# SparkJiao/llama-pipeline-parallel

Measured on AMD Instinct MI355X. Metric: tokens/sec (whole node), LLaMA-65B PP=8 seq4096 at 1/2/4/8 MI355X, higher is better.
Workload: dtype bf16; 1 GPU; model=llama-65b, measured_model=llama-65b-shaped 10-layer slice (10/80 layers), global_batch=64, seq_len=4096, parallelism=pp1, num_layers=10, micro_batch_size=4, grad_accum_steps=16

## Files before the change

### lpp_amd/ops/csrc/attention_bwd.hip

```cpp
#include "common.h"
#include "attn_order.h"

namespace lpp {

typedef __attribute__((ext_vector_type(8))) short bf16x8;
typedef __attribute__((ext_vector_type(16))) float f32x16;
typedef __attribute__((ext_vector_type(2))) int int2v;

constexpr int AB_D = 128;

__device__ __forceinline__ int bswz(int row, int col_elem) {
  return row * 256 + ((col_elem * 2) ^ ((row & 15) << 4));
}
__device__ __forceinline__ unsigned cvt_pk_bf16_(float lo, float hi) {
  unsigned r;
  asm("v_cvt_pk_bf16_f32 %0, %1, %2" : "=v"(r) : "v"(lo), "v"(hi));
  return r;
}
__device__ __forceinline__ float bf2f_(short s) {
  union { unsigned u; float f; } cv;
  cv.u = ((unsigned)(unsigned short)s) << 16;
  return cv.f;
}
__device__ __forceinline__ short f2bf_(float f) {
  __hip_bfloat16 h = __float2bfloat16(f);
  return *reinterpret_cast<short*>(&h);
}

__device__ __forceinline__ void quad_transpose(const bf16x8& v, int st_r, int out[4]) {
#pragma unroll
  for (int k = 0; k < 4; ++k) out[k] = reinterpret_cast<const int*>(&v)[k];
  {
    int t0 = __shfl_xor(out[(st_r & 1) ^ 1], 16);
    int t1 = __shfl_xor(out[((st_r & 1) ^ 1) | 2], 16);
    if (st_r & 1) { out[0] = t0; out[2] = t1; } else { out[1] = t0; out[3] = t1; }
  }
  {
    int lo = (st_r & 2) ? 0 : 2;
    int t0 = __shfl_xor(out[lo], 32);
    int t1 = __shfl_xor(out[lo + 1], 32);
    out[lo] = t0; out[lo + 1] = t1;
  }
}

__device__ __forceinline__ int tswz(int d, int r) {
  return (d * 64 + (r ^ ((((d >> 3) ^ d) & 7) << 3))) * 2;
}

__device__ __forceinline__ void write_transposed(char* img, int r0, int d0,
                                                 const int dw[4]) {
#pragma unroll
  for (int e = 0; e < 2; ++e) {
    const int d = d0 + e;
    unsigned w01 = e ? (((unsigned)dw[0] >> 16) | ((unsigned)dw[1] & 0xffff0000u))
                     : (((unsigned)dw[0] & 0xffffu) | ((unsigned)dw[1] << 16));
    unsigned w23 = e ? (((unsigned)dw[2] >> 16) | ((unsigned)dw[3] & 0xffff0000u))
                     : (((unsigned)dw[2] & 0xffffu) | ((unsigned)dw[3] << 16));
    int2v pair = {(int)w01, (int)w23};
    *reinterpret_cast<int2v*>(img + tswz(d, r0)) = pair;
  }
}

__device__ __forceinline__ void pack_pair(const float p[16], bf16x8 out[2]) {
#pragma unroll
  for (int ksl = 0; ksl < 2; ++ksl) {
    const float* pr = &p[8 * ksl];
    const unsigned x1 = cvt_pk_bf16_(pr[0], pr[1]);
    const unsigned x2 = cvt_pk_bf16_(pr[2], pr[3]);
    const unsigned y1 = cvt_pk_bf16_(pr[4], pr[5]);
    const unsigned y2 = cvt_pk_bf16_(pr[6], pr[7]);
    const int2v a = __builtin_amdgcn_permlane32_swap((int)x1, (int)y1, false, false);
    const int2v b = __builtin_amdgcn_permlane32_swap((int)x2, (int)y2, false, false);
    int w[4] = {a[0], b[0], a[1], b[1]};
    out[ksl] = *reinterpret_cast<const bf16x8*>(w);
  }
}

__global__ __launch_bounds__(256) void attn_bwd_delta_kernel(
    const short* __restrict__ dO, const short* __restrict__ O,
    float* __restrict__ delta, int64_t rows, int S, int H) {
  const int lg = threadIdx.x & 15;
  const int grp = (blockIdx.x * 256 + (int)threadIdx.x) >> 4;
  const int64_t stride = ((int64_t)gridDim.x * 256) >> 4;
  for (int64_t r = grp; r < rows; r += stride) {
    const bf16x8 d8 = *reinterpret_cast<const bf16x8*>(&dO[r * AB_D + lg * 8]);
    const bf16x8 o8 = *reinterpret_cast<const bf16x8*>(&O[r * AB_D + lg * 8]);
    float acc = 0.f;
#pragma unroll
    for (int j = 0; j < 8; ++j) acc += bf2f_(d8[j]) * bf2f_(o8[j]);
#pragma unroll
    for (int m = 1; m < 16; m <<= 1) acc += __shfl_xor(acc, m);
    if (lg == 0) {
      const int h = (int)(r % H);
      const int64_t bs = r / H;
      const int s = (int)(bs % S);
      const int64_t b = bs / S;
      delta[(b * H + h) * S + s] = acc;
    }
  }
}

constexpr int DQ_QW = 32, DQ_WAVES = 8, DQ_QB = 256, DQ_KVB = 64;

template <bool DBUF>
__global__ __launch_bounds__(512, 2) void attn_bwd_dq_kernel(
    const short* __restrict__ Q, const short* __restrict__ K,
    const short* __restrict__ V, const short* __restrict__ dO,
    const float* __restrict__ LSE2, const float* __restrict__ Delta,
    short* __restrict__ dQ,
    int B, int S, int H, int HKV, float c, float scale,
    int order_mode, int order_G) {
  extern __shared__ __attribute__((aligned(16))) char smem[];
  constexpr int NB = DBUF ? 2 : 1;
  auto k_lds = [&](int buf) -> char* { return smem + (DBUF ? buf : 0) * 16384; };
  auto v_lds = [&](int buf) -> char* {
    return smem + NB * 16384 + (DBUF ? buf : 0) * 16384; };
  auto kt_lds = [&](int buf) -> char* {
    return smem + 2 * NB * 16384 + (DBUF ? buf : 0) * 16384; };

  const int tid = threadIdx.x;
  const int wid = tid >> 6;
  const int lane = tid & 63;
  const int lq = lane & 31;
  const int hi2 = lane >> 5;

  const AttnBlock ob = attn_block_order(blockIdx.x, (S + DQ_QB - 1) / DQ_QB, B * H,
                                        order_G, ATTN_ORDER_FWD_DQ, order_mode);
  const int qblk = ob.blk;
  const int b = ob.head / H;
  const int h = ob.head % H;
  const int hkv = h / (H / HKV);
  const int64_t sHD = (int64_t)H * AB_D;
  const int64_t sHkvD = (int64_t)HKV * AB_D;
  const int64_t q_base = (((int64_t)b * S) * H + h) * AB_D;
  const int64_t kv_base = (((int64_t)b * S) * HKV + hkv) * AB_D;
  const int64_t ld_base = ((int64_t)b * H + h) * S;

  const int qw0 = qblk * DQ_QB + wid * DQ_QW;
  const int qrow = qw0 + lq;

  bf16x8 qf[8], dof[8];
  {
    const int64_t rb = q_base + (int64_t)min(qrow, S - 1) * sHD;
#pragma unroll
    for (int dc = 0; dc < 8; ++dc) {
      qf[dc] = *reinterpret_cast<const bf16x8*>(&Q[rb + dc * 16 + hi2 * 8]);
      dof[dc] = *reinterpret_cast<const bf16x8*>(&dO[rb + dc * 16 + hi2 * 8]);
    }
  }
  const float Lq = LSE2[ld_base + min(qrow, S - 1)];
  const float Dq = Delta[ld_base + min(qrow, S - 1)];

  const int st_r = lane >> 4;
  const int st_c = 8 * (lane & 15);
  const int kv_end = min(S, (qblk + 1) * DQ_QB);

  auto ld_tile = [&](int kv0, int pass, bf16x8& kreg, bf16x8& vreg) {
    const int row = min(kv0 + 4 * wid + 32 * pass + st_r, S - 1);
    const int64_t rb = kv_base + (int64_t)row * sHkvD + st_c;
    kreg = *reinterpret_cast<const bf16x8*>(&K[rb]);
    vreg = *reinterpret_cast<const bf16x8*>(&V[rb]);
  };
  auto write_tile = [&](int buf, int pass, bf16x8 kreg, bf16x8 vreg) {
    const int r = 4 * wid + 32 * pass + st_r;
    *reinterpret_cast<bf16x8*>(k_lds(buf) + bswz(r, st_c)) = kreg;
    *reinterpret_cast<bf16x8*>(v_lds(buf) + bswz(r, st_c)) = vreg;
    int dw[4];
    quad_transpose(kreg, st_r, dw);
    write_transposed(kt_lds(buf), 4 * wid + 32 * pass, st_c + 2 * st_r, dw);
  };

  f32x16 dq_acc[4];
#pragma unroll
  for (int dt = 0; dt < 4; ++dt)
#pragma unroll
    for (int r = 0; r < 16; ++r) dq_acc[dt][r] = 0.f;

  bf16x8 kreg0, kreg1, vreg0, vreg1;
  ld_tile(0, 0, kreg0, vreg0);
  ld_tile(0, 1, kreg1, vreg1);
  write_tile(0, 0, kreg0, vreg0);
  write_tile(0, 1, kreg1, vreg1);
  if (DBUF && DQ_KVB < kv_end) {
    ld_tile(DQ_KVB, 0, kreg0, vreg0);
    ld_tile(DQ_KVB, 1, kreg1, vreg1);
  }
  __syncthreads();

  for (int kv0 = 0, cur = 0; kv0 < kv_end; kv0 += DQ_KVB, cur ^= 1) {
    const bool have_next = kv0 + DQ_KVB < kv_end;
    if (DBUF) {
      if (have_next) {
        write_tile(cur ^ 1, 0, kreg0, vreg0);
        write_tile(cur ^ 1, 1, kreg1, vreg1);
        if (kv0 + 2 * DQ_KVB < kv_end) {
          ld_tile(kv0 + 2 * DQ_KVB, 0, kreg0, vreg0);
          ld_tile(kv0 + 2 * DQ_KVB, 1, kreg1, vreg1);
        }
      }
    } else if (have_next) {
      ld_tile(kv0 + DQ_KVB, 0, kreg0, vreg0);
      ld_tile(kv0 + DQ_KVB, 1, kreg1, vreg1);
    }

    if (kv0 < qw0 + DQ_QW) {
      f32x16 st[2], dpt[2];
#pragma unroll
      for (int t2 = 0; t2 < 2; ++t2)
#pragma unroll
        for (int r = 0; r < 16; ++r) { st[t2][r] = 0.f; dpt[t2][r] = 0.f; }
      __builtin_amdgcn_s_setprio(1);
#pragma unroll
      for (int dc = 0; dc < 8; ++dc) {
#pragma unroll
        for (int t2 = 0; t2 < 2; ++t2) {
          const bf16x8 ak = *reinterpret_cast<const bf16x8*>(
              k_lds(cur) + bswz(t2 * 32 + lq, dc * 16 + hi2 * 8));
          const bf16x8 av = *reinterpret_cast<const bf16x8*>(
              v_lds(cur) + bswz(t2 * 32 + lq, dc * 16 + hi2 * 8));
          st[t2] = __builtin_amdgcn_mfma_f32_32x32x16_bf16(ak, qf[dc], st[t2], 0, 0, 0);
          dpt[t2] = __builtin_amdgcn_mfma_f32_32x32x16_bf16(av, dof[dc], dpt[t2], 0, 0, 0);
        }
      }
      __builtin_amdgcn_s_setprio(0);

      const bool need_mask = (kv0 + DQ_KVB > qw0) || (kv0 + DQ_KVB > S);
      float ds[32];
#pragma unroll
      for (int t2 = 0; t2 < 2; ++t2)
#pragma unroll
        for (int r = 0; r < 16; ++r) {
          bool ok = true;
          if (need_mask) {
            const int kv = kv0 + t2 * 32 + (r & 3) + 8 * (r >> 2) + 4 * hi2;
            ok = (kv <= qrow) && (kv < S);
          }
          const float p = ok ? exp2f(fmaf(st[t2][r], c, -Lq)) : 0.f;
          ds[t2 * 16 + r] = p * (dpt[t2][r] - Dq);
        }

      bf16x8 dsa[4];
      pack_pair(&ds[0], &dsa[0]);
      pack_pair(&ds[16], &dsa[2]);

      __builtin_amdgcn_s_setprio(1);
#pragma unroll
      for (int dt = 0; dt < 4; ++dt) {
        const int d = dt * 32 + lq;
#pragma unroll
        for (int ks = 0; ks < 4; ++ks) {
          const bf16x8 bk = *reinterpret_cast<const bf16x8*>(
              kt_lds(cur) + tswz(d, ks * 16 + hi2 * 8));
          dq_acc[dt] = __builtin_amdgcn_mfma_f32_32x32x16_bf16(dsa[ks], bk, dq_acc[dt], 0, 0, 0);
        }
      }
      __builtin_amdgcn_s_setprio(0);
    }

    if (!DBUF && have_next) {
      __syncthreads();
      write_tile(0, 0, kreg0, vreg0);
      write_tile(0, 1, kreg1, vreg1);
    }
    __syncthreads();
  }

#pragma unroll
  for (int r = 0; r < 16; ++r) {
    const int row = qw0 + (r & 3) + 8 * (r >> 2) + 4 * hi2;
    if (row >= S) continue;
    const int64_t rb = q_base + (int64_t)row * sHD;
#pragma unroll
    for (int dt = 0; dt < 4; ++dt) dQ[rb + dt * 32 + lq] = f2bf_(dq_acc[dt][r] * scale);
  }
}

constexpr int KV_KW = 16, KV_WG = 128, KV_QT = 64;
constexpr int TS40 = 40;

typedef __attribute__((ext_vector_type(4))) float f32x4;


__device__ __forceinline__ bf16x8 pack_frag16(const float p[2][4], int hi4_odd) {
  unsigned X0 = cvt_pk_bf16_(p[0][0], p[0][1]);
  unsigned Y0 = cvt_pk_bf16_(p[0][2], p[0][3]);
  unsigned X1 = cvt_pk_bf16_(p[1][0], p[1][1]);
  unsigned Y1 = cvt_pk_bf16_(p[1][2], p[1][3]);
  const int2v ax = __builtin_amdgcn_permlane32_swap((int)X0, (int)X1, false, false);
  const int2v cx = __builtin_amdgcn_permlane16_swap(ax[0], ax[0], false, false);
  const int2v cpx = __builtin_amdgcn_permlane16_swap(ax[1], ax[1], false, false);
  const int2v ay = __builtin_amdgcn_permlane32_swap((int)Y0, (int)Y1, false, false);
  const int2v cy = __builtin_amdgcn_permlane16_swap(ay[0], ay[0], false, false);
  const int2v cpy = __builtin_amdgcn_permlane16_swap(ay[1], ay[1], false, false);
  int w[4];
  w[0] = hi4_odd ? cpx[0] : ax[0];
  w[1] = hi4_odd ? cpy[0] : ay[0];
  w[2] = hi4_odd ? ax[1] : cx[1];
  w[3] = hi4_odd ? ay[1] : cy[1];
  return *reinterpret_cast<const bf16x8*>(w);
}

template <bool DBUF>
__global__ __launch_bounds__(512, 2) void attn_bwd_dkdv_kernel(
    const short* __restrict__ Q, const short* __restrict__ K,
    const short* __restrict__ V, const short* __restrict__ dO,
    const float* __restrict__ LSE2, const float* __restrict__ Delta,
    short* __restrict__ dK, short* __restrict__ dV,
    int B, int S, int H, int HKV, float c, float scale,
    int order_mode, int order_G) {
  extern __shared__ __attribute__((aligned(16))) char smem[];
  constexpr int NB = DBUF ? 2 : 1;
  auto q_lds = [&](int buf) -> char* { return smem + (DBUF ? buf : 0) * 16384; };
  auto do_lds = [&](int buf) -> char* {
    return smem + NB * 16384 + (DBUF ? buf : 0) * 16384; };
  auto qt_lds = [&](int buf) -> char* {
    return smem + 2 * NB * 16384 + (DBUF ? buf : 0) * 16384; };
  auto dot_lds = [&](int buf) -> char* {
    return smem + 3 * NB * 16384 + (DBUF ? buf : 0) * 16384; };
  auto l_buf = [&](int buf) -> float* {
    return reinterpret_cast<float*>(smem + 4 * NB * 16384) + (DBUF ? buf : 0) * 64; };
  auto d_buf = [&](int buf) -> float* {
    return reinterpret_cast<float*>(smem + 4 * NB * 16384 + NB * 256) +
           (DBUF ? buf : 0) * 64; };


  const int tid = threadIdx.x;
  const int wid = tid >> 6;
  const int lane = tid & 63;
  const int l16 = lane & 15;
  const int hi4 = (lane >> 4) & 3;

  const AttnBlock ob = attn_block_order(blockIdx.x, (S + KV_WG - 1) / KV_WG, B * HKV,
                                        order_G, ATTN_ORDER_DKDV, order_mode);
  const int kvblk = ob.blk;
  const int b = ob.head / HKV;
  const int hkv = ob.head % HKV;
  const int G = H / HKV;
  const int64_t sHD = (int64_t)H * AB_D;
  const int64_t sHkvD = (int64_t)HKV * AB_D;
  const int64_t kv_base = (((int64_t)b * S) * HKV + hkv) * AB_D;

  const int kvw0 = kvblk * KV_WG + wid * KV_KW;
  const int kvrow = kvw0 + l16;

  bf16x8 kf[4], vf[4];
  {
    const int64_t rb = kv_base + (int64_t)min(kvrow, S - 1) * sHkvD;
#pragma unroll
    for (int dc = 0; dc < 4; ++dc) {
      kf[dc] = *reinterpret_cast<const bf16x8*>(&K[rb + dc * 32 + hi4 * 8]);
      vf[dc] = *reinterpret_cast<const bf16x8*>(&V[rb + dc * 32 + hi4 * 8]);
    }
  }

  f32x4 dv_acc[8], dk_acc[8];
#pragma unroll
  for (int dt = 0; dt < 8; ++dt)
#pragma unroll
    for (int r = 0; r < 4; ++r) { dv_acc[dt][r] = 0.f; dk_acc[dt][r] = 0.f; }

  const int st_r = (lane >> 4) & 3;
  const int st_c = 8 * (lane & 15);
  const int qstart = kvblk * KV_WG;

  for (int g = 0; g < G; ++g) {
    const int h = hkv * G + g;
    const int64_t q_base = (((int64_t)b * S) * H + h) * AB_D;
    const int64_t ld_base = ((int64_t)b * H + h) * S;

    auto ld_tile = [&](int qt0, int pass, bf16x8& qreg, bf16x8& dreg) {
      const int row = min(qt0 + 4 * wid + 32 * pass + st_r, S - 1);
      const int64_t rb = q_base + (int64_t)row * sHD + st_c;
      qreg = *reinterpret_cast<const bf16x8*>(&Q[rb]);
      dreg = *reinterpret_cast<const bf16x8*>(&dO[rb]);
    };
    auto write_tile = [&](int buf, int qt0, int pass, bf16x8 qreg, bf16x8 dreg) {
      const int r = 4 * wid + 32 * pass + st_r;
      *reinterpret_cast<bf16x8*>(q_lds(buf) + bswz(r, st_c)) = qreg;
      *reinterpret_cast<bf16x8*>(do_lds(buf) + bswz(r, st_c)) = dreg;
      int dw[4];
      quad_transpose(qreg, st_r, dw);
      write_transposed(qt_lds(buf), r - st_r, st_c + 2 * st_r, dw);
      quad_transpose(dreg, st_r, dw);
      write_transposed(dot_lds(buf), r - st_r, st_c + 2 * st_r, dw);
      if (pass == 0 && tid < 128) {
        const int qi = min(qt0 + (tid & 63), S - 1);
        if (tid < 64) l_buf(buf)[tid] = LSE2[ld_base + qi];
        else d_buf(buf)[tid & 63] = Delta[ld_base + qi];
      }
    };

    bf16x8 qreg0, dreg0, qreg1, dreg1;
    ld_tile(qstart, 0, qreg0, dreg0);
    ld_tile(qstart, 1, qreg1, dreg1);
    write_tile(0, qstart, 0, qreg0, dreg0);
    write_tile(0, qstart, 1, qreg1, dreg1);
    if (DBUF && qstart + KV_QT < S) {
      ld_tile(qstart + KV_QT, 0, qreg0, dreg0);
      ld_tile(qstart + KV_QT, 1, qreg1, dreg1);
    }
    __syncthreads();

    for (int qt0 = qstart, cur = 0; qt0 < S; qt0 += KV_QT, cur ^= 1) {
      const bool have_next = qt0 + KV_QT < S;
      if (DBUF) {
        if (have_next) {
          write_tile(cur ^ 1, qt0 + KV_QT, 0, qreg0, dreg0);
          write_tile(cur ^ 1, qt0 + KV_QT, 1, qreg1, dreg1);
          if (qt0 + 2 * KV_QT < S) {
            ld_tile(qt0 + 2 * KV_QT, 0, qreg0, dreg0);
            ld_tile(qt0 + 2 * KV_QT, 1, qreg1, dreg1);
          }
        }
      } else if (have_next) {
        ld_tile(qt0 + KV_QT, 0, qreg0, dreg0);
        ld_tile(qt0 + KV_QT, 1, qreg1, dreg1);
      }

      if (qt0 + KV_QT - 1 >= kvw0) {
#pragma unroll
        for (int half = 0; half < 2; ++half) {
          const int qh0 = qt0 + half * 32;
          if (qh0 + 31 < kvw0) continue;
          f32x4 st[2], dpt[2];
#pragma unroll
          for (int qs = 0; qs < 2; ++qs)
#pragma unroll
            for (int r = 0; r < 4; ++r) { st[qs][r] = 0.f; dpt[qs][r] = 0.f; }
          __builtin_amdgcn_s_setprio(1);
#pragma unroll
          for (int dc = 0; dc < 4; ++dc) {
#pragma unroll
            for (int qs = 0; qs < 2; ++qs) {
              const bf16x8 aq = *reinterpret_cast<const bf16x8*>(
                  q_lds(cur) + bswz(half * 32 + qs * 16 + l16, dc * 32 + hi4 * 8));
              const bf16x8 ad = *reinterpret_cast<const bf16x8*>(
                  do_lds(cur) + bswz(half * 32 + qs * 16 + l16, dc * 32 + hi4 * 8));
              st[qs] = __builtin_amdgcn_mfma_f32_16x16x32_bf16(aq, kf[dc], st[qs], 0, 0, 0);
              dpt[qs] = __builtin_amdgcn_mfma_f32_16x16x32_bf16(ad, vf[dc], dpt[qs], 0, 0, 0);
            }
          }
          __builtin_amdgcn_s_setprio(0);

          const bool need_mask = (qh0 < kvw0 + KV_KW) || (qh0 + 32 > S);
          float p[2][4], ds[2][4];
#pragma unroll
          for (int qs = 0; qs < 2; ++qs) {
            const int q0 = half * 32 + qs * 16 + hi4 * 4;
            const f32x4 Lr = *reinterpret_cast<const f32x4*>(&l_buf(cur)[q0]);
            const f32x4 Dr = *reinterpret_cast<const f32x4*>(&d_buf(cur)[q0]);
#pragma unroll
            for (int r = 0; r < 4; ++r) {
              bool ok = (kvrow < S);
              if (need_mask) {
                const int q = qt0 + q0 + r;
                ok = ok && (q >= kvrow) && (q < S);
              }
              p[qs][r] = ok ? exp2f(fmaf(st[qs][r], c, -Lr[r])) : 0.f;
              ds[qs][r] = p[qs][r] * (dpt[qs][r] - Dr[r]);
            }
          }

          const bf16x8 pa = pack_frag16(p, hi4 & 1);
          const bf16x8 dsa = pack_frag16(ds, hi4 & 1);

          __builtin_amdgcn_s_setprio(1);
#pragma unroll
          for (int dt = 0; dt < 8; ++dt) {
            const int d = dt * 16 + l16;
            const bf16x8 bd = *reinterpret_cast<const bf16x8*>(
                dot_lds(cur) + tswz(d, half * 32 + hi4 * 8));
            const bf16x8 bq = *reinterpret_cast<const bf16x8*>(
                qt_lds(cur) + tswz(d, half * 32 + hi4 * 8));
            dv_acc[dt] = __builtin_amdgcn_mfma_f32_16x16x32_bf16(pa, bd, dv_acc[dt], 0, 0, 0);
            dk_acc[dt] = __builtin_amdgcn_mfma_f32_16x16x32_bf16(dsa, bq, dk_acc[dt], 0, 0, 0);
          }
          __builtin_amdgcn_s_setprio(0);
        }
      }

      if (!DBUF && have_next) {
        __syncthreads();
        write_tile(0, qt0 + KV_QT, 0, qreg0, dreg0);
        write_tile(0, qt0 + KV_QT, 1, qreg1, dreg1);
      }
      __syncthreads();
    }
    __syncthreads();
  }

#pragma unroll
  for (int r = 0; r < 4; ++r) {
    const int row = kvw0 + hi4 * 4 + r;
    if (row >= S) continue;
    const int64_t rb = kv_base + (int64_t)row * sHkvD;
#pragma unroll
    for (int dt = 0; dt < 8; ++dt) {
      dV[rb + dt * 16 + l16] = f2bf_(dv_acc[dt][r]);
      dK[rb + dt * 16 + l16] = f2bf_(dk_acc[dt][r] * scale);
    }
  }
}

static bool attn_dbuf() {
  static const bool dbuf = [] {
    const char* e = getenv("LPP_ATTN_DBUF");
    return e && e[0] == '1';
  }();
  return dbuf;
}

void launch_attn_fwd(const at::Tensor& q, const at::Tensor& k, const at::Tensor& v,
                     at::Tensor& o, at::Tensor& lse2, int order_mode, int order_G);

static void launch_attn_bwd_delta(const at::Tensor& dO, const at::Tensor& o,
                                  at::Tensor& delta) {
  const int B = dO.size(0), S = dO.size(1), H = dO.size(2);
  const int64_t rows = (int64_t)B * S * H;
  const int grid = grid_for(rows * 16, 256);
  hipLaunchKernelGGL(attn_bwd_delta_kernel, dim3(grid), dim3(256), 0, current_stream(),
                     (const short*)dO.data_ptr(), (const short*)o.data_ptr(),
                     delta.data_ptr<float>(), rows, S, H);
  LPP_CHECK_HIP(hipGetLastError());
}

static void launch_attn_bwd_dq(const at::Tensor& dO, const at::Tensor& q,
                               const at::Tensor& k, const at::Tensor& v,
                               const at::Tensor& lse2, const at::Tensor& delta,
                               at::Tensor& dq, int order_mode, int order_G) {
  const int B = q.size(0), S = q.size(1), H = q.size(2);
  const int HKV = k.size(2);
  const float scale = 1.0f / std::sqrt((float)AB_D);
  const float c = scale * 1.4426950408889634f;
  const bool dbuf = attn_dbuf();
  const int qblocks = (S + DQ_QB - 1) / DQ_QB;
  if (order_G <= 0) order_G = attn_order_group(dbuf ? 32 : 64, qblocks);
  const size_t lds = dbuf ? 98304 : 49152;
  auto kfn = dbuf ? attn_bwd_dq_kernel<true> : attn_bwd_dq_kernel<false>;
  hipLaunchKernelGGL(kfn, dim3(qblocks * B * H), dim3(512), lds,
                     current_stream(), (const short*)q.data_ptr(), (const short*)k.data_ptr(),
                     (const short*)v.data_ptr(), (const short*)dO.data_ptr(),
                     lse2.data_ptr<float>(), delta.data_ptr<float>(),
                     (short*)dq.data_ptr(), B, S, H, HKV, c, scale, order_mode, order_G);
  LPP_CHECK_HIP(hipGetLastError());
}

static void launch_attn_bwd_dkdv(const at::Tensor& dO, const at::Tensor& q,
                                 const at::Tensor& k, const at::Tensor& v,
                                 const at::Tensor& lse2, const at::Tensor& delta,
                                 at::Tensor& dk, at::Tensor& dv, int order_mode,
                                 int order_G) {
  const int B = q.size(0), S = q.size(1), H = q.size(2);
  const int HKV = k.size(2);
  const float scale = 1.0f / std::sqrt((float)AB_D);
  const float c = scale * 1.4426950408889634f;
  const bool dbuf = attn_dbuf();
  const int kvblocks = (S + KV_WG - 1) / KV_WG;
  if (order_G <= 0) order_G = attn_order_group(dbuf ? 32 : 64, kvblocks);
  const size_t lds = dbuf ? (131072 + 1024) : (65536 + 512);
  auto kfn = dbuf ? attn_bwd_dkdv_kernel<true> : attn_bwd_dkdv_kernel<false>;
  hipLaunchKernelGGL(kfn, dim3(kvblocks * B * HKV), dim3(512), lds,
                     current_stream(), (const short*)q.data_ptr(), (const short*)k.data_ptr(),
                     (const short*)v.data_ptr(), (const short*)dO.data_ptr(),
                     lse2.data_ptr<float>(), delta.data_ptr<float>(),
                     (short*)dk.data_ptr(), (short*)dv.data_ptr(), B, S, H, HKV, c,
                     scale, order_mode, order_G);
  LPP_CHECK_HIP(hipGetLastError());
}

}

static void attention_bwd_check(const at::Tensor& dO, const at::Tensor& q,
                                const at::Tensor& k, const at::Tensor& v,
                                const at::Tensor& o, const at::Tensor& lse2) {
  TORCH_CHECK(q.is_cuda() && q.scalar_type() == at::kBFloat16, "attention_bwd: bf16 only");
  TORCH_CHECK(q.dim() == 4 && q.size(3) == lpp::AB_D, "attention_bwd: [B,S,H,128] required");
  TORCH_CHECK(dO.is_contiguous() && q.is_contiguous() && k.is_contiguous() &&
              v.is_contiguous() && o.is_contiguous() && lse2.is_contiguous());
  TORCH_CHECK(q.size(2) % k.size(2) == 0);
}

std::vector<at::Tensor> attention_bwd(at::Tensor dO, at::Tensor q, at::Tensor k,
                                      at::Tensor v, at::Tensor o, at::Tensor lse2) {
  attention_bwd_check(dO, q, k, v, o, lse2);
  const int B = q.size(0), S = q.size(1), H = q.size(2);
  auto delta = at::empty({B, H, S}, q.options().dtype(at::kFloat));
  lpp::launch_attn_bwd_delta(dO, o, delta);
  auto dq = at::empty_like(q);
  auto dk = at::empty_like(k);
  auto dv = at::empty_like(v);
  const int mode = lpp::attn_order_mode();
  lpp::launch_attn_bwd_dq(dO, q, k, v, lse2, delta, dq, mode ? lpp::ATTN_MODE1_DQ : 0, 0);
  lpp::launch_attn_bwd_dkdv(dO, q, k, v, lse2, delta, dk, dv,
                            mode ? lpp::ATTN_MODE1_DKDV : 0, 0);
  return {dq, dk, dv};
}

std::vector<double> attention_time_kernel(std::string kernel, at::Tensor dO, at::Tensor q,
                                          at::Tensor k, at::Tensor v, at::Tensor o,
                                          at::Tensor lse2, int64_t mode, int64_t G,
                                          int64_t warmup, int64_t reps) {
  attention_bwd_check(dO, q, k, v, o, lse2);
  TORCH_CHECK(mode == 0 || mode == 1, "attention_time_kernel: mode 0 or 1");
  TORCH_CHECK(kernel == "fwd" || kernel == "dq" || kernel == "dkdv",
              "attention_time_kernel: kernel is fwd, dq or dkdv");
  const int B = q.size(0), S = q.size(1), H = q.size(2);
  auto delta = at::empty({B, H, S}, q.options().dtype(at::kFloat));
  lpp::launch_attn_bwd_delta(dO, o, delta);
  auto o2 = at::empty_like(q), dq = at::empty_like(q);
  auto lse_out = at::empty_like(lse2);
  auto dk = at::empty_like(k), dv = at::empty_like(v);
  auto launch = [&] {
    if (kernel == "fwd") lpp::launch_attn_fwd(q, k, v, o2, lse_out, (int)mode, (int)G);
    else if (kernel == "dq")
      lpp::launch_attn_bwd_dq(dO, q, k, v, lse2, delta, dq, (int)mode, (int)G);
    else lpp::launch_attn_bwd_dkdv(dO, q, k, v, lse2, delta, dk, dv, (int)mode, (int)G);
  };
  auto stream = lpp::current_stream();
  hipEvent_t e0, e1;
  LPP_CHECK_HIP(hipEventCreate(&e0));
  LPP_CHECK_HIP(hipEventCreate(&e1));
  for (int64_t i = 0; i < warmup; ++i) launch();
  std::vector<double> ms;
  for (int64_t i = 0; i < reps; ++i) {
    LPP_CHECK_HIP(hipEventRecord(e0, stream));
    launch();
    LPP_CHECK_HIP(hipEventRecord(e1, stream));
    LPP_CHECK_HIP(hipEventSynchronize(e1));
    float t = 0.f;
    LPP_CHECK_HIP(hipEventElapsedTime(&t, e0, e1));
    ms.push_back(t);
  }
  LPP_CHECK_HIP(hipEventDestroy(e0));
  LPP_CHECK_HIP(hipEventDestroy(e1));
  return ms;
}
```

### lpp_amd/ops/csrc/attention_fwd.hip

```cpp
#include "common.h"
#include "attn_order.h"

namespace lpp {

typedef __attribute__((ext_vector_type(8))) short bf16x8;
typedef __attribute__((ext_vector_type(16))) float f32x16;
typedef __attribute__((ext_vector_type(2))) int int2v;

constexpr int AF_D = 128;
constexpr int AF_QW = 32;
constexpr int AF_WAVES = 8;
constexpr int AF_QB = AF_QW * AF_WAVES;
constexpr int AF_KVB = 64;
constexpr float AF_THR = 8.0f;

__device__ __forceinline__ int kswz(int row, int col_elem) {
  return row * 256 + ((col_elem * 2) ^ ((row & 15) << 4));
}
__device__ __forceinline__ int vswz(int d, int kv) {
  return (d * 64 + (kv ^ ((((d >> 3) ^ d) & 7) << 3))) * 2;
}

__device__ __forceinline__ unsigned cvt_pk_bf16(float lo, float hi) {
  unsigned r;
  asm("v_cvt_pk_bf16_f32 %0, %1, %2" : "=v"(r) : "v"(lo), "v"(hi));
  return r;
}
__device__ __forceinline__ float as_f(int v) { return __int_as_float(v); }
__device__ __forceinline__ int as_i(float v) { return __float_as_int(v); }

__global__ __launch_bounds__(512, 2) void attn_fwd_kernel(
    const short* __restrict__ Q, const short* __restrict__ K,
    const short* __restrict__ V, short* __restrict__ O, float* __restrict__ LSE2,
    int B, int S, int H, int HKV, float c ,
    int order_mode, int order_G) {
  extern __shared__ __attribute__((aligned(16))) char smem[];
  auto k_lds = [&](int buf) -> char* { return smem + buf * 16384; };
  auto vt_lds = [&](int buf) -> char* { return smem + 32768 + buf * 16384; };

  const int tid = threadIdx.x;
  const int wid = tid >> 6;
  const int lane = tid & 63;
  const int lq = lane & 31;
  const int hi2 = lane >> 5;

  const AttnBlock ob = attn_block_order(blockIdx.x, (S + AF_QB - 1) / AF_QB, B * H,
                                        order_G, ATTN_ORDER_FWD_DQ, order_mode);
  const int qblk = ob.blk;
  const int bh = ob.head;
  const int b = bh / H;
  const int h = bh % H;
  const int hkv = h / (H / HKV);

  const int64_t sHD = (int64_t)H * AF_D;
  const int64_t sHkvD = (int64_t)HKV * AF_D;
  const int64_t q_base = (((int64_t)b * S) * H + h) * AF_D;
  const int64_t kv_base = (((int64_t)b * S) * HKV + hkv) * AF_D;

  const int qw0 = qblk * AF_QB + wid * AF_QW;
  const int qrow = qw0 + lq;

  bf16x8 qf[8];
  {
    const int64_t rb = q_base + (int64_t)min(qrow, S - 1) * sHD;
#pragma unroll
    for (int dc = 0; dc < 8; ++dc)
      qf[dc] = *reinterpret_cast<const bf16x8*>(&Q[rb + dc * 16 + hi2 * 8]);
  }

  const int st_r = (lane >> 4);
  const int st_c = 8 * (lane & 15);

  const int kv_end = min(S, (qblk + 1) * AF_QB);

  auto ld_tile = [&](int kv0, int pass, bf16x8& kreg, bf16x8& vreg) {
    const int row = min(kv0 + 4 * wid + 32 * pass + st_r, S - 1);
    const int64_t rb = kv_base + (int64_t)row * sHkvD + st_c;
    kreg = *reinterpret_cast<const bf16x8*>(&K[rb]);
    vreg = *reinterpret_cast<const bf16x8*>(&V[rb]);
  };

  auto write_tile = [&](int buf, int pass, bf16x8 kreg, bf16x8 vreg) {
    const int r = 4 * wid + 32 * pass + st_r;
    *reinterpret_cast<bf16x8*>(k_lds(buf) + kswz(r, st_c)) = kreg;
    int dw[4];
#pragma unroll
    for (int k = 0; k < 4; ++k) dw[k] = reinterpret_cast<const int*>(&vreg)[k];
    {
      int t0 = __shfl_xor(dw[(st_r & 1) ^ 1], 16);
      int t1 = __shfl_xor(dw[((st_r & 1) ^ 1) | 2], 16);
      if (st_r & 1) { dw[0] = t0; dw[2] = t1; } else { dw[1] = t0; dw[3] = t1; }
    }
    {
      int lo = (st_r & 2) ? 0 : 2, hi = lo + 1;
      int t0 = __shfl_xor(dw[lo], 32);
      int t1 = __shfl_xor(dw[hi], 32);
      dw[lo] = t0; dw[hi] = t1;
    }
    const int r0 = 4 * wid + 32 * pass;
    const int d0 = st_c + 2 * st_r;
#pragma unroll
    for (int e = 0; e < 2; ++e) {
      const int d = d0 + e;
      unsigned w01 = e ? (((unsigned)dw[0] >> 16) | ((unsigned)dw[1] & 0xffff0000u))
                       : (((unsigned)dw[0] & 0xffffu) | ((unsigned)dw[1] << 16));
      unsigned w23 = e ? (((unsigned)dw[2] >> 16) | ((unsigned)dw[3] & 0xffff0000u))
                       : (((unsigned)dw[2] & 0xffffu) | ((unsigned)dw[3] << 16));
      int2v pair = {(int)w01, (int)w23};
      *reinterpret_cast<int2v*>(vt_lds(buf) + vswz(d, r0)) = pair;
    }
  };

  f32x16 o_acc[4];
#pragma unroll
  for (int dt = 0; dt < 4; ++dt)
#pragma unroll
    for (int r = 0; r < 16; ++r) o_acc[dt][r] = 0.f;
  float m_run = -INFINITY, l_run = 0.f;

  bf16x8 kreg0, kreg1, vreg0, vreg1;
  ld_tile(0, 0, kreg0, vreg0);
  ld_tile(0, 1, kreg1, vreg1);
  write_tile(0, 0, kreg0, vreg0);
  write_tile(0, 1, kreg1, vreg1);
  if (AF_KVB < kv_end) {
    ld_tile(AF_KVB, 0, kreg0, vreg0);
    ld_tile(AF_KVB, 1, kreg1, vreg1);
  }
  __syncthreads();

  for (int kv0 = 0, cur = 0; kv0 < kv_end; kv0 += AF_KVB, cur ^= 1) {
    const bool have_next = kv0 + AF_KVB < kv_end;
    if (have_next) {
      write_tile(cur ^ 1, 0, kreg0, vreg0);
      write_tile(cur ^ 1, 1, kreg1, vreg1);
      if (kv0 + 2 * AF_KVB < kv_end) {
        ld_tile(kv0 + 2 * AF_KVB, 0, kreg0, vreg0);
        ld_tile(kv0 + 2 * AF_KVB, 1, kreg1, vreg1);
      }
    }

    if (kv0 < qw0 + AF_QW) {
      f32x16 st[2];
#pragma unroll
      for (int t2 = 0; t2 < 2; ++t2)
#pragma unroll
        for (int r = 0; r < 16; ++r) st[t2][r] = 0.f;
      __builtin_amdgcn_s_setprio(1);
#pragma unroll
      for (int dc = 0; dc < 8; ++dc) {
#pragma unroll
        for (int t2 = 0; t2 < 2; ++t2) {
          const bf16x8 kf = *reinterpret_cast<const bf16x8*>(
              k_lds(cur) + kswz(t2 * 32 + lq, dc * 16 + hi2 * 8));
          st[t2] = __builtin_amdgcn_mfma_f32_32x32x16_bf16(kf, qf[dc], st[t2], 0, 0, 0);
        }
      }
      __builtin_amdgcn_s_setprio(0);

      float ms[32];
      const bool need_mask = (kv0 + AF_KVB > qw0) || (kv0 + AF_KVB > S);
#pragma unroll
      for (int t2 = 0; t2 < 2; ++t2)
#pragma unroll
        for (int r = 0; r < 16; ++r) {
          float v = st[t2][r];
          if (need_mask) {
            const int kv = kv0 + t2 * 32 + (r & 3) + 8 * (r >> 2) + 4 * hi2;
            if (kv > qrow || kv >= S) v = -INFINITY;
          }
          ms[t2 * 16 + r] = v;
        }

      float pmax = ms[0];
#pragma unroll
      for (int i = 1; i < 32; ++i) pmax = fmaxf(pmax, ms[i]);
      {
        int2v sw = __builtin_amdgcn_permlane32_swap(as_i(pmax), as_i(pmax), false, false);
        pmax = fmaxf(pmax, as_f(hi2 ? sw[0] : sw[1]));
      }
      const float rm2 = pmax * c;

      float m_new = m_run;
      if (__any(rm2 > m_run + AF_THR)) {
        m_new = fmaxf(m_run, rm2);
        const float alpha = (m_run == -INFINITY) ? 0.f : exp2f(m_run - m_new);
        l_run *= alpha;
#pragma unroll
        for (int r = 0; r < 16; ++r) {
          const int src = (r & 3) + 8 * (r >> 2) + 4 * hi2;
          const float ar = as_f(__builtin_amdgcn_ds_bpermute(src * 4, as_i(alpha)));
#pragma unroll
          for (int dt = 0; dt < 4; ++dt) o_acc[dt][r] *= ar;
        }
        m_run = m_new;
      }

      float p[32];
      float ps = 0.f;
#pragma unroll
      for (int i = 0; i < 32; ++i) {
        p[i] = exp2f(fmaf(ms[i], c, -m_new));
        ps += p[i];
      }
      {
        int2v sw = __builtin_amdgcn_permlane32_swap(as_i(ps), as_i(ps), false, false);
        ps += as_f(hi2 ? sw[0] : sw[1]);
      }
      l_run += ps;

      bf16x8 pa[4];
#pragma unroll
      for (int t2 = 0; t2 < 2; ++t2)
#pragma unroll
        for (int ksl = 0; ksl < 2; ++ksl) {
          const float* pr = &p[t2 * 16 + 8 * ksl];
          const unsigned x1 = cvt_pk_bf16(pr[0], pr[1]);
          const unsigned x2 = cvt_pk_bf16(pr[2], pr[3]);
          const unsigned y1 = cvt_pk_bf16(pr[4], pr[5]);
          const unsigned y2 = cvt_pk_bf16(pr[6], pr[7]);
          const int2v a = __builtin_amdgcn_permlane32_swap((int)x1, (int)y1, false, false);
          const int2v bsw = __builtin_amdgcn_permlane32_swap((int)x2, (int)y2, false, false);
          int w[4] = {a[0], bsw[0], a[1], bsw[1]};
          pa[t2 * 2 + ksl] = *reinterpret_cast<const bf16x8*>(w);
        }

      __builtin_amdgcn_s_setprio(1);
#pragma unroll
      for (int dt = 0; dt < 4; ++dt) {
        const int d = dt * 32 + lq;
#pragma unroll
        for (int ks = 0; ks < 4; ++ks) {
          const bf16x8 bv = *reinterpret_cast<const bf16x8*>(
              vt_lds(cur) + vswz(d, ks * 16 + hi2 * 8));
          o_acc[dt] = __builtin_amdgcn_mfma_f32_32x32x16_bf16(pa[ks], bv, o_acc[dt], 0, 0, 0);
        }
      }
      __builtin_amdgcn_s_setprio(0);
    }

    __syncthreads();
  }

  const float invl = (l_run > 0.f) ? 1.f / l_run : 0.f;
#pragma unroll
  for (int r = 0; r < 16; ++r) {
    const int rq = (r & 3) + 8 * (r >> 2) + 4 * hi2;
    const float ir = as_f(__builtin_amdgcn_ds_bpermute(rq * 4, as_i(invl)));
    const int row = qw0 + rq;
    if (row >= S) continue;
    const int64_t rb = q_base + (int64_t)row * sHD;
#pragma unroll
    for (int dt = 0; dt < 4; ++dt) {
      __hip_bfloat16 hv = __float2bfloat16(o_acc[dt][r] * ir);
      O[rb + dt * 32 + lq] = *reinterpret_cast<short*>(&hv);
    }
  }
  if (hi2 == 0 && qrow < S)
    LSE2[((int64_t)b * H + h) * S + qrow] = m_run + log2f(l_run);
}

static int g_order_mode = [] {
  const char* e = getenv("LPP_ATTN_ORDER");
  return (e && e[0] == '0') ? 0 : 1;
}();

int attn_order_mode() { return g_order_mode; }

void launch_attn_fwd(const at::Tensor& q, const at::Tensor& k, const at::Tensor& v,
                     at::Tensor& o, at::Tensor& lse2, int order_mode, int order_G) {
  const int B = q.size(0), S = q.size(1), H = q.size(2);
  const int HKV = k.size(2);
  const float scale = 1.0f / std::sqrt((float)AF_D);
  const float c = scale * 1.4426950408889634f;
  const int qblocks = (S + AF_QB - 1) / AF_QB;
  if (order_G <= 0) order_G = attn_order_group(64, qblocks);
  const size_t lds = 65536;
  hipLaunchKernelGGL(attn_fwd_kernel, dim3(qblocks * B * H), dim3(512), lds,
                     current_stream(), (const short*)q.data_ptr(),
                     (const short*)k.data_ptr(), (const short*)v.data_ptr(),
                     (short*)o.data_ptr(), lse2.data_ptr<float>(), B, S, H, HKV, c,
                     order_mode, order_G);
  LPP_CHECK_HIP(hipGetLastError());
}

}

std::vector<at::Tensor> attention_fwd(at::Tensor q, at::Tensor k, at::Tensor v) {
  TORCH_CHECK(q.is_cuda() && q.scalar_type() == at::kBFloat16, "attention_fwd: bf16 only");
  TORCH_CHECK(q.dim() == 4 && q.size(3) == lpp::AF_D, "attention_fwd: [B,S,H,128] required");
  TORCH_CHECK(q.is_contiguous() && k.is_contiguous() && v.is_contiguous());
  const int B = q.size(0), S = q.size(1), H = q.size(2);
  const int HKV = k.size(2);
  TORCH_CHECK(H % HKV == 0);
  auto o = at::empty_like(q);
  auto lse2 = at::empty({B, H, S}, q.options().dtype(at::kFloat));
  lpp::launch_attn_fwd(q, k, v, o, lse2,
                       lpp::attn_order_mode() ? lpp::ATTN_MODE1_FWD : 0, 0);
  return {o, lse2};
}

void attention_set_block_order(int64_t mode) {
  TORCH_CHECK(mode == 0 || mode == 1, "attention_set_block_order: mode 0 or 1");
  lpp::g_order_mode = (int)mode;
}

int64_t attention_get_block_order() { return lpp::g_order_mode; }

at::Tensor attention_block_order(int64_t kind, int64_t nblk, int64_t nheads, int64_t G,
                                 int64_t mode) {
  TORCH_CHECK(kind == 0 || kind == 1, "attention_block_order: kind 0 (fwd/dQ) or 1 (dK/dV)");
  TORCH_CHECK(mode == 0 || mode == 1, "attention_block_order: mode 0 or 1");
  TORCH_CHECK(nblk >= 1 && nheads >= 1 && nblk * nheads < (int64_t)1 << 30 && G >= 1);
  G = std::min(G, nheads);
  const int n = (int)(nblk * nheads);
  auto out = at::empty({n, 2}, at::TensorOptions().dtype(at::kInt));
  int* p = out.data_ptr<int>();
  for (int L = 0; L < n; ++L) {
    const lpp::AttnBlock ob =
        lpp::attn_block_order(L, (int)nblk, (int)nheads, (int)G, (int)kind, (int)mode);
    p[2 * L] = ob.blk;
    p[2 * L + 1] = ob.head;
  }
  return out;
}
```

### lpp_amd/ops/csrc/attn_order.h

```cpp
#pragma once

#if defined(__HIP__) || defined(__CUDACC__)
#define LPP_HD __host__ __device__
#else
#define LPP_HD
#endif

namespace lpp {

constexpr int ATTN_XCDS = 8;

enum AttnOrderKind : int {
  ATTN_ORDER_FWD_DQ = 0,
  ATTN_ORDER_DKDV = 1,
};

struct AttnBlock {
  int blk;
  int head;
};

LPP_HD inline AttnBlock attn_block_order(int L, int nblk, int nheads, int G, int kind,
                                         int mode) {
  if (mode == 0) return {L % nblk, L / nblk};
  const int n = nblk * nheads;
  const int xcd = L % ATTN_XCDS;
  const int q = n / ATTN_XCDS, r = n % ATTN_XCDS;
  const int j = (xcd < r ? xcd * (q + 1) : r * (q + 1) + (xcd - r) * q) + L / ATTN_XCDS;
  if (G < 1) G = 1;
  if (G > nheads) G = nheads;
  const int grp = j / (G * nblk), rem = j % (G * nblk);
  const int Gl = G < nheads - grp * G ? G : nheads - grp * G;
  const int rank = rem / Gl;
  return {kind == ATTN_ORDER_FWD_DQ ? nblk - 1 - rank : rank, grp * G + rem % Gl};
}

inline int attn_order_group(int resident_per_xcd, int nblk) {
  const int g = (resident_per_xcd + nblk - 1) / nblk;
  return g < 1 ? 1 : g;
}

int attn_order_mode();

constexpr int ATTN_MODE1_FWD = 1;
constexpr int ATTN_MODE1_DQ = 1;
constexpr int ATTN_MODE1_DKDV = 1;

}
```

Baseline: 22910 tokens/s.

## Make double-buffered LDS the only attention backward path and restructure dQ loop

Drops the env-gated single-buffer variant so the dQ and dKdV backward kernels always double-buffer their K/V and Q/dO tiles in LDS, overlapping global loads with compute. The change also splits the dQ inner loop per 32-row sub-tile to cut register pressure, adds unmasked fast paths for the softmax recompute, and uses readfirstlane on the wave id. The block-order group size changes to 4×32 waves per XCD for the forward and backward kernels. The larger LDS footprint (96KB and 129KB) may lower occupancy compared with the previous single-buffer default.

Result: faster. 23340 tokens/s, median of 6 (+1.9%).

```diff
diff --git a/lpp_amd/ops/csrc/attention_bwd.hip b/lpp_amd/ops/csrc/attention_bwd.hip
--- a/lpp_amd/ops/csrc/attention_bwd.hip
+++ b/lpp_amd/ops/csrc/attention_bwd.hip
@@ -102,7 +102,6 @@
 
 constexpr int DQ_QW = 32, DQ_WAVES = 8, DQ_QB = 256, DQ_KVB = 64;
 
-template <bool DBUF>
 __global__ __launch_bounds__(512, 2) void attn_bwd_dq_kernel(
     const short* __restrict__ Q, const short* __restrict__ K,
     const short* __restrict__ V, const short* __restrict__ dO,
@@ -111,15 +110,12 @@
     int B, int S, int H, int HKV, float c, float scale,
     int order_mode, int order_G) {
   extern __shared__ __attribute__((aligned(16))) char smem[];
-  constexpr int NB = DBUF ? 2 : 1;
-  auto k_lds = [&](int buf) -> char* { return smem + (DBUF ? buf : 0) * 16384; };
-  auto v_lds = [&](int buf) -> char* {
-    return smem + NB * 16384 + (DBUF ? buf : 0) * 16384; };
-  auto kt_lds = [&](int buf) -> char* {
-    return smem + 2 * NB * 16384 + (DBUF ? buf : 0) * 16384; };
+  auto k_lds = [&](int buf) -> char* { return smem + buf * 16384; };
+  auto v_lds = [&](int buf) -> char* { return smem + 32768 + buf * 16384; };
+  auto kt_lds = [&](int buf) -> char* { return smem + 65536 + buf * 16384; };
 
   const int tid = threadIdx.x;
-  const int wid = tid >> 6;
+  const int wid = __builtin_amdgcn_readfirstlane(tid >> 6);
   const int lane = tid & 63;
   const int lq = lane & 31;
   const int hi2 = lane >> 5;
@@ -181,87 +177,74 @@
   ld_tile(0, 1, kreg1, vreg1);
   write_tile(0, 0, kreg0, vreg0);
   write_tile(0, 1, kreg1, vreg1);
-  if (DBUF && DQ_KVB < kv_end) {
+  if (DQ_KVB < kv_end) {
     ld_tile(DQ_KVB, 0, kreg0, vreg0);
     ld_tile(DQ_KVB, 1, kreg1, vreg1);
   }
   __syncthreads();
 
   for (int kv0 = 0, cur = 0; kv0 < kv_end; kv0 += DQ_KVB, cur ^= 1) {
-    const bool have_next = kv0 + DQ_KVB < kv_end;
-    if (DBUF) {
-      if (have_next) {
-        write_tile(cur ^ 1, 0, kreg0, vreg0);
-        write_tile(cur ^ 1, 1, kreg1, vreg1);
-        if (kv0 + 2 * DQ_KVB < kv_end) {
-          ld_tile(kv0 + 2 * DQ_KVB, 0, kreg0, vreg0);
-          ld_tile(kv0 + 2 * DQ_KVB, 1, kreg1, vreg1);
-        }
+    if (kv0 + DQ_KVB < kv_end) {
+      write_tile(cur ^ 1, 0, kreg0, vreg0);
+      write_tile(cur ^ 1, 1, kreg1, vreg1);
+      if (kv0 + 2 * DQ_KVB < kv_end) {
+        ld_tile(kv0 + 2 * DQ_KVB, 0, kreg0, vreg0);
+        ld_tile(kv0 + 2 * DQ_KVB, 1, kreg1, vreg1);
       }
-    } else if (have_next) {
-      ld_tile(kv0 + DQ_KVB, 0, kreg0, vreg0);
-      ld_tile(kv0 + DQ_KVB, 1, kreg1, vreg1);
     }
 
     if (kv0 < qw0 + DQ_QW) {
-      f32x16 st[2], dpt[2];
-#pragma unroll
-      for (int t2 = 0; t2 < 2; ++t2)
-#pragma unroll
-        for (int r = 0; r < 16; ++r) { st[t2][r] = 0.f; dpt[t2][r] = 0.f; }
-      __builtin_amdgcn_s_setprio(1);
-#pragma unroll
-      for (int dc = 0; dc < 8; ++dc) {
-#pragma unroll
-        for (int t2 = 0; t2 < 2; ++t2) {
+      const bool need_mask = (kv0 + DQ_KVB > qw0) || (kv0 + DQ_KVB > S);
+#pragma unroll
+      for (int t2 = 0; t2 < 2; ++t2) {
+        f32x16 st, dpt;
+#pragma unroll
+        for (int r = 0; r < 16; ++r) { st[r] = 0.f; dpt[r] = 0.f; }
+        __builtin_amdgcn_s_setprio(1);
+#pragma unroll
+        for (int dc = 0; dc < 8; ++dc) {
           const bf16x8 ak = *reinterpret_cast<const bf16x8*>(
               k_lds(cur) + bswz(t2 * 32 + lq, dc * 16 + hi2 * 8));
           const bf16x8 av = *reinterpret_cast<const bf16x8*>(
               v_lds(cur) + bswz(t2 * 32 + lq, dc * 16 + hi2 * 8));
-          st[t2] = __builtin_amdgcn_mfma_f32_32x32x16_bf16(ak, qf[dc], st[t2], 0, 0, 0);
-          dpt[t2] = __builtin_amdgcn_mfma_f32_32x32x16_bf16(av, dof[dc], dpt[t2], 0, 0, 0);
+          st = __builtin_amdgcn_mfma_f32_32x32x16_bf16(ak, qf[dc], st, 0, 0, 0);
+          dpt = __builtin_amdgcn_mfma_f32_32x32x16_bf16(av, dof[dc], dpt, 0, 0, 0);
         }
+        __builtin_amdgcn_s_setprio(0);
+
+        float ds[16];
+        if (need_mask) {
+#pragma unroll
+          for (int r = 0; r < 16; ++r) {
+            const int kv = kv0 + t2 * 32 + (r & 3) + 8 * (r >> 2) + 4 * hi2;
+            const bool ok = (kv <= qrow) && (kv < S);
+            const float e = exp2f(fmaf(st[r], c, -Lq));
+            ds[r] = (ok ? e : 0.f) * (dpt[r] - Dq);
+          }
+        } else {
+#pragma unroll
+          for (int r = 0; r < 16; ++r)
+            ds[r] = exp2f(fmaf(st[r], c, -Lq)) * (dpt[r] - Dq);
+        }
+
+        bf16x8 dsa[2];
+        pack_pair(ds, dsa);
+
+        __builtin_amdgcn_s_setprio(1);
+#pragma unroll
+        for (int dt = 0; dt < 4; ++dt) {
+          const int d = dt * 32 + lq;
+#pragma unroll
+          for (int ks = 0; ks < 2; ++ks) {
+            const bf16x8 bk = *reinterpret_cast<const bf16x8*>(
+                kt_lds(cur) + tswz(d, (2 * t2 + ks) * 16 + hi2 * 8));
+            dq_acc[dt] = __builtin_amdgcn_mfma_f32_32x32x16_bf16(dsa[ks], bk, dq_acc[dt], 0, 0, 0);
+          }
+        }
+        __builtin_amdgcn_s_setprio(0);
       }
-      __builtin_amdgcn_s_setprio(0);
-
-      const bool need_mask = (kv0 + DQ_KVB > qw0) || (kv0 + DQ_KVB > S);
-      float ds[32];
-#pragma unroll
-      for (int t2 = 0; t2 < 2; ++t2)
-#pragma unroll
-        for (int r = 0; r < 16; ++r) {
-          bool ok = true;
-          if (need_mask) {
-            const int kv = kv0 + t2 * 32 + (r & 3) + 8 * (r >> 2) + 4 * hi2;
-            ok = (kv <= qrow) && (kv < S);
-          }
-          const float p = ok ? exp2f(fmaf(st[t2][r], c, -Lq)) : 0.f;
-          ds[t2 * 16 + r] = p * (dpt[t2][r] - Dq);
-        }
-
-      bf16x8 dsa[4];
-      pack_pair(&ds[0], &dsa[0]);
-      pack_pair(&ds[16], &dsa[2]);
-
-      __builtin_amdgcn_s_setprio(1);
-#pragma unroll
-      for (int dt = 0; dt < 4; ++dt) {
-        const int d = dt * 32 + lq;
-#pragma unroll
-        for (int ks = 0; ks < 4; ++ks) {
-          const bf16x8 bk = *reinterpret_cast<const bf16x8*>(
-              kt_lds(cur) + tswz(d, ks * 16 + hi2 * 8));
-          dq_acc[dt] = __builtin_amdgcn_mfma_f32_32x32x16_bf16(dsa[ks], bk, dq_acc[dt], 0, 0, 0);
-        }
-      }
-      __builtin_amdgcn_s_setprio(0);
-    }
-
-    if (!DBUF && have_next) {
-      __syncthreads();
-      write_tile(0, 0, kreg0, vreg0);
-      write_tile(0, 1, kreg1, vreg1);
-    }
+    }
+
     __syncthreads();
   }
 
@@ -300,7 +283,6 @@
   return *reinterpret_cast<const bf16x8*>(w);
 }
 
-template <bool DBUF>
 __global__ __launch_bounds__(512, 2) void attn_bwd_dkdv_kernel(
     const short* __restrict__ Q, const short* __restrict__ K,
     const short* __restrict__ V, const short* __restrict__ dO,
@@ -309,23 +291,17 @@
     int B, int S, int H, int HKV, float c, float scale,
     int order_mode, int order_G) {
   extern __shared__ __attribute__((aligned(16))) char smem[];
-  constexpr int NB = DBUF ? 2 : 1;
-  auto q_lds = [&](int buf) -> char* { return smem + (DBUF ? buf : 0) * 16384; };
-  auto do_lds = [&](int buf) -> char* {
-    return smem + NB * 16384 + (DBUF ? buf : 0) * 16384; };
-  auto qt_lds = [&](int buf) -> char* {
-    return smem + 2 * NB * 16384 + (DBUF ? buf : 0) * 16384; };
-  auto dot_lds = [&](int buf) -> char* {
-    return smem + 3 * NB * 16384 + (DBUF ? buf : 0) * 16384; };
+  auto q_lds = [&](int buf) -> char* { return smem + buf * 16384; };
+  auto do_lds = [&](int buf) -> char* { return smem + 32768 + buf * 16384; };
+  auto qt_lds = [&](int buf) -> char* { return smem + 65536 + buf * 16384; };
+  auto dot_lds = [&](int buf) -> char* { return smem + 98304 + buf * 16384; };
   auto l_buf = [&](int buf) -> float* {
-    return reinterpret_cast<float*>(smem + 4 * NB * 16384) + (DBUF ? buf : 0) * 64; };
+    return reinterpret_cast<float*>(smem + 131072) + buf * 64; };
   auto d_buf = [&](int buf) -> float* {
-    return reinterpret_cast<float*>(smem + 4 * NB * 16384 + NB * 256) +
-           (DBUF ? buf : 0) * 64; };
-
+    return reinterpret_cast<float*>(smem + 131072 + 512) + buf * 64; };
 
   const int tid = threadIdx.x;
-  const int wid = tid >> 6;
+  const int wid = __builtin_amdgcn_readfirstlane(tid >> 6);
   const int lane = tid & 63;
   const int l16 = lane & 15;
   const int hi4 = (lane >> 4) & 3;
@@ -395,26 +371,20 @@
     ld_tile(qstart, 1, qreg1, dreg1);
     write_tile(0, qstart, 0, qreg0, dreg0);
     write_tile(0, qstart, 1, qreg1, dreg1);
-    if (DBUF && qstart + KV_QT < S) {
+    if (qstart + KV_QT < S) {
       ld_tile(qstart + KV_QT, 0, qreg0, dreg0);
       ld_tile(qstart + KV_QT, 1, qreg1, dreg1);
     }
     __syncthreads();
 
     for (int qt0 = qstart, cur = 0; qt0 < S; qt0 += KV_QT, cur ^= 1) {
-      const bool have_next = qt0 + KV_QT < S;
-      if (DBUF) {
-        if (have_next) {
-          write_tile(cur ^ 1, qt0 + KV_QT, 0, qreg0, dreg0);
-          write_tile(cur ^ 1, qt0 + KV_QT, 1, qreg1, dreg1);
-          if (qt0 + 2 * KV_QT < S) {
-            ld_tile(qt0 + 2 * KV_QT, 0, qreg0, dreg0);
-            ld_tile(qt0 + 2 * KV_QT, 1, qreg1, dreg1);
-          }
+      if (qt0 + KV_QT < S) {
+        write_tile(cur ^ 1, qt0 + KV_QT, 0, qreg0, dreg0);
+        write_tile(cur ^ 1, qt0 + KV_QT, 1, qreg1, dreg1);
+        if (qt0 + 2 * KV_QT < S) {
+          ld_tile(qt0 + 2 * KV_QT, 0, qreg0, dreg0);
+          ld_tile(qt0 + 2 * KV_QT, 1, qreg1, dreg1);
         }
-      } else if (have_next) {
-        ld_tile(qt0 + KV_QT, 0, qreg0, dreg0);
-        ld_tile(qt0 + KV_QT, 1, qreg1, dreg1);
       }
 
       if (qt0 + KV_QT - 1 >= kvw0) {
@@ -449,15 +419,21 @@
             const int q0 = half * 32 + qs * 16 + hi4 * 4;
             const f32x4 Lr = *reinterpret_cast<const f32x4*>(&l_buf(cur)[q0]);
             const f32x4 Dr = *reinterpret_cast<const f32x4*>(&d_buf(cur)[q0]);
-#pragma unroll
-            for (int r = 0; r < 4; ++r) {
-              bool ok = (kvrow < S);
-              if (need_mask) {
+            if (need_mask) {
+#pragma unroll
+              for (int r = 0; r < 4; ++r) {
                 const int q = qt0 + q0 + r;
-                ok = ok && (q >= kvrow) && (q < S);
+                const bool ok = (kvrow < S) && (q >= kvrow) && (q < S);
+                const float e = exp2f(fmaf(st[qs][r], c, -Lr[r]));
+                p[qs][r] = ok ? e : 0.f;
+                ds[qs][r] = p[qs][r] * (dpt[qs][r] - Dr[r]);
               }
-              p[qs][r] = ok ? exp2f(fmaf(st[qs][r], c, -Lr[r])) : 0.f;
-              ds[qs][r] = p[qs][r] * (dpt[qs][r] - Dr[r]);
+            } else {
+#pragma unroll
+              for (int r = 0; r < 4; ++r) {
+                p[qs][r] = exp2f(fmaf(st[qs][r], c, -Lr[r]));
+                ds[qs][r] = p[qs][r] * (dpt[qs][r] - Dr[r]);
+              }
             }
           }
 
@@ -479,11 +455,6 @@
         }
       }
 
-      if (!DBUF && have_next) {
-        __syncthreads();
-        write_tile(0, qt0 + KV_QT, 0, qreg0, dreg0);
-        write_tile(0, qt0 + KV_QT, 1, qreg1, dreg1);
-      }
       __syncthreads();
     }
     __syncthreads();
@@ -500,14 +471,6 @@
       dK[rb + dt * 16 + l16] = f2bf_(dk_acc[dt][r] * scale);
     }
   }
-}
-
-static bool attn_dbuf() {
-  static const bool dbuf = [] {
-    const char* e = getenv("LPP_ATTN_DBUF");
-    return e && e[0] == '1';
-  }();
-  return dbuf;
 }
 
 void launch_attn_fwd(const at::Tensor& q, const at::Tensor& k, const at::Tensor& v,
@@ -532,12 +495,11 @@
   const int HKV = k.size(2);
   const float scale = 1.0f / std::sqrt((float)AB_D);
   const float c = scale * 1.4426950408889634f;
-  const bool dbuf = attn_dbuf();
   const int qblocks = (S + DQ_QB - 1) / DQ_QB;
-  if (order_G <= 0) order_G = attn_order_group(dbuf ? 32 : 64, qblocks);
-  const size_t lds = dbuf ? 98304 : 49152;
-  auto kfn = dbuf ? attn_bwd_dq_kernel<true> : attn_bwd_dq_kernel<false>;
-  hipLaunchKernelGGL(kfn, dim3(qblocks * B * H), dim3(512), lds,
+  if (order_G <= 0)
+    order_G = attn_order_group(ATTN_GROUP_WAVES * ATTN_RESIDENT_PER_XCD, qblocks);
+  const size_t lds = 98304;
+  hipLaunchKernelGGL(attn_bwd_dq_kernel, dim3(qblocks * B * H), dim3(512), lds,
                      current_stream(), (const short*)q.data_ptr(), (const short*)k.data_ptr(),
                      (const short*)v.data_ptr(), (const short*)dO.data_ptr(),
                      lse2.data_ptr<float>(), delta.data_ptr<float>(),
@@ -554,12 +516,11 @@
   const int HKV = k.size(2);
   const float scale = 1.0f / std::sqrt((float)AB_D);
   const float c = scale * 1.4426950408889634f;
-  const bool dbuf = attn_dbuf();
   const int kvblocks = (S + KV_WG - 1) / KV_WG;
-  if (order_G <= 0) order_G = attn_order_group(dbuf ? 32 : 64, kvblocks);
-  const size_t lds = dbuf ? (131072 + 1024) : (65536 + 512);
-  auto kfn = dbuf ? attn_bwd_dkdv_kernel<true> : attn_bwd_dkdv_kernel<false>;
-  hipLaunchKernelGGL(kfn, dim3(kvblocks * B * HKV), dim3(512), lds,
+  if (order_G <= 0)
+    order_G = attn_order_group(ATTN_GROUP_WAVES * ATTN_RESIDENT_PER_XCD, kvblocks);
+  const size_t lds = 131072 + 1024;
+  hipLaunchKernelGGL(attn_bwd_dkdv_kernel, dim3(kvblocks * B * HKV), dim3(512), lds,
                      current_stream(), (const short*)q.data_ptr(), (const short*)k.data_ptr(),
                      (const short*)v.data_ptr(), (const short*)dO.data_ptr(),
                      lse2.data_ptr<float>(), delta.data_ptr<float>(),
diff --git a/lpp_amd/ops/csrc/attention_fwd.hip b/lpp_amd/ops/csrc/attention_fwd.hip
--- a/lpp_amd/ops/csrc/attention_fwd.hip
+++ b/lpp_amd/ops/csrc/attention_fwd.hip
@@ -274,7 +274,8 @@
   const float scale = 1.0f / std::sqrt((float)AF_D);
   const float c = scale * 1.4426950408889634f;
   const int qblocks = (S + AF_QB - 1) / AF_QB;
-  if (order_G <= 0) order_G = attn_order_group(64, qblocks);
+  if (order_G <= 0)
+    order_G = attn_order_group(ATTN_GROUP_WAVES * ATTN_RESIDENT_PER_XCD, qblocks);
   const size_t lds = 65536;
   hipLaunchKernelGGL(attn_fwd_kernel, dim3(qblocks * B * H), dim3(512), lds,
                      current_stream(), (const short*)q.data_ptr(),
diff --git a/lpp_amd/ops/csrc/attn_order.h b/lpp_amd/ops/csrc/attn_order.h
--- a/lpp_amd/ops/csrc/attn_order.h
+++ b/lpp_amd/ops/csrc/attn_order.h
@@ -35,6 +35,9 @@
   return {kind == ATTN_ORDER_FWD_DQ ? nblk - 1 - rank : rank, grp * G + rem % Gl};
 }
 
+constexpr int ATTN_RESIDENT_PER_XCD = 32;
+constexpr int ATTN_GROUP_WAVES = 4;
+
 inline int attn_order_group(int resident_per_xcd, int nblk) {
   const int g = (resident_per_xcd + nblk - 1) / nblk;
   return g < 1 ? 1 : g;
```
